# BVE-Reborn/rend3

Hardware: NVIDIA H100
Metric: culled objects/s (fused frustum cull + object-uniform bake) (higher is better)
Workload: dtype f32

## Files before the change

### __graft_entry__.py

```python
import os
import subprocess
import sys

ROOT = os.path.dirname(os.path.abspath(__file__))
CSRC = os.path.join(ROOT, "rend3_b200", "csrc")
OUT = os.path.join(ROOT, "rend3_b200", "librend3_b200.so")
NVCC = os.environ.get("NVCC", "/usr/local/cuda/bin/nvcc")
HOST_CXX = "/usr/bin/g++" if os.path.exists("/usr/bin/g++") else "g++"

SOURCES = [
    ("r3_ctx.cu", ["-fmad=false"]),
    ("r3_cull_bake.cu", ["-fmad=false"]),
    ("r3_tri_cull.cu", ["-fmad=false"]),
    ("r3_raster.cu", ["-fmad=false"]),
    ("r3_shade.cu", []),
    ("r3_batching.cpp", ["-fmad=false"]),
    ("r3_gpu_batching.cu", ["-fmad=false"]),
    ("r3_skinning.cu", ["-fmad=false"]),
    ("r3_animation.cu", ["-fmad=false"]),
    ("r3_object_transforms.cu", ["-fmad=false"]),
    ("r3_mesh_deform.cu", ["-fmad=false"]),
    ("r3_lights.cu", ["-fmad=false"]),
    ("r3_peer.cu", ["-fmad=false"]),
    ("r3_texture_write.cu", ["-fmad=false"]),
]
GENCODE = ["-gencode", "arch=compute_90a,code=sm_90a"]
COMMON = [
    "-std=c++17", "-O3", "-lineinfo", *GENCODE,
    "-ccbin", HOST_CXX, "-Xcompiler", "-fPIC,-fvisibility=hidden,-Wall,-Wno-unused-function",
    "-prec-div=true", "-prec-sqrt=true",
]


def _stale(target, deps):
    if not os.path.exists(target):
        return True
    t = os.path.getmtime(target)
    return any(os.path.getmtime(d) > t for d in deps if os.path.exists(d))


def build(verbose: bool = False) -> None:
    headers = [os.path.join(CSRC, "r3_common.cuh"), os.path.join(CSRC, "r3_scan.cuh"), os.path.join(CSRC, "r3_radix.cuh"), os.path.join(CSRC, "r3_texture.cuh"),
               os.path.join(ROOT, "include", "rend3_b200.h"), os.path.join(ROOT, "include", "r3_layouts.h"), os.path.join(ROOT, "include", "r3_anim_check.h")]
    objs = []
    if os.path.exists(NVCC):
        for src, extra in SOURCES:
            s = os.path.join(CSRC, src)
            o = os.path.join(CSRC, os.path.splitext(src)[0] + ".o")
            objs.append(o)
            if _stale(o, [s] + headers):
                cmd = [NVCC, "-x", "cu", "-c", s, "-o", o] + COMMON + extra + (["-Xptxas", "-v"] if verbose else [])
                r = subprocess.run(cmd, capture_output=True, text=True)
                if verbose or r.returncode != 0:
                    sys.stderr.write(r.stdout + r.stderr)
                if r.returncode != 0:
                    raise RuntimeError(f"nvcc failed on {src}")
        if _stale(OUT, objs):
            cmd = [NVCC, "-shared", "-o", OUT] + objs + GENCODE + ["-ccbin", HOST_CXX, "-lcudart"]
            r = subprocess.run(cmd, capture_output=True, text=True)
            if r.returncode != 0:
                sys.stderr.write(r.stdout + r.stderr)
                raise RuntimeError("link failed")
    elif not os.path.exists(OUT):
        raise RuntimeError("nvcc not found and no prebuilt librend3_b200.so")
    host_src, host_bin = os.path.join(ROOT, "rend3_b200", "host", "r3_frame.cpp"), os.path.join(ROOT, "rend3_b200", "host", "r3_frame")
    if _stale(host_bin, [host_src, OUT, os.path.join(ROOT, "include", "rend3_b200.hpp")] + headers):
        cmd = [HOST_CXX, "-std=c++17", "-O2", "-Wall", "-I", os.path.join(ROOT, "include"), host_src, "-o", host_bin,
               "-L", os.path.join(ROOT, "rend3_b200"), "-lrend3_b200", "-Wl,-rpath,$ORIGIN/.."]
        r = subprocess.run(cmd, capture_output=True, text=True)
        if r.returncode != 0:
            sys.stderr.write(r.stdout + r.stderr)
            raise RuntimeError("host driver build failed")
    sys.path.insert(0, ROOT)
    import oracle
    import oracle.anim
    import oracle.objanim
    import oracle.lights
    import oracle.objtransforms
    import oracle.points

    oracle.build()
    oracle.anim.build()
    oracle.objanim.build()
    oracle.lights.build()
    oracle.objtransforms.build()
    oracle.points.build()
    import rend3_b200


def smoke() -> None:
    sys.path.insert(0, ROOT)
    import numpy as np

    import oracle
    from rend3_b200 import load_cuda_backend
    from rend3_b200.scenes import cube_field_scene
    from rend3_b200.routines import BaseRenderGraph, BaseRenderGraphSettings

    results = {}
    for name, backend in (("cuda", load_cuda_backend(0, parity_target=True)), ("oracle", oracle.load_oracle_backend())):
        ev = cube_field_scene(n_objects=300, seed=7, resolution=(256, 144))
        graph = BaseRenderGraph(backend)
        graph.add_to_graph(ev, (256, 144), 1, BaseRenderGraphSettings(clear_color=(0.1, 0.05, 0.1, 1.0)))
        results[name] = (backend.readback_visible(0xFFFFFFFF).copy(), backend.readback_hdr_f32().copy(), backend.readback_depth().copy())
    vis_c, hdr_c, dep_c = results["cuda"]
    vis_o, hdr_o, dep_o = results["oracle"]
    assert np.array_equal(vis_c, vis_o), "visible-object list differs from the oracle"
    assert np.array_equal(dep_c, dep_o), "depth buffer differs from the oracle"
    err = np.abs(hdr_c - hdr_o) / np.maximum(1.0, np.abs(hdr_o))
    assert err.max() <= 1e-4, f"shaded pixels differ from the oracle by {err.max()}"
    print(f"smoke ok: {len(vis_c)} visible objects, max pixel error {err.max():.2e}")


if __name__ == "__main__":
    build(verbose="-v" in sys.argv)
    print("built", OUT)
```

### rend3_b200/csrc/r3_cull_bake.cu

```cuda
#include <cstdlib>
#include <type_traits>

#include "r3_common.cuh"
#include "r3_scan.cuh"

namespace {

constexpr int CB_THREADS = 256;
constexpr int CB_WARPS = CB_THREADS / 32;
constexpr int CB_WT = 4;
constexpr int CB_CTA_OBJECTS = CB_WARPS * CB_WT * 32;
constexpr int CP_THREADS = 1024;
constexpr int CP_OBJECTS = CP_THREADS * 32;
constexpr int CP_CTAS_PER_TILE = CP_OBJECTS / CB_CTA_OBJECTS;

struct CullBakeParams {
    float view[16];
    float view_proj[16];
    float frustum[5][4];
    uint32_t object_count;
};
struct DeviceCameraParams {
    const r3_camera_header* cam;
    uint32_t object_count;
};
constexpr int CAM_FLOATS = 52;

__global__ void __launch_bounds__(256) split_objects_kernel(const float4* __restrict__ objects, uint32_t n, float* __restrict__ rows_xyz, float* __restrict__ rows_w,
                                                            float4* __restrict__ spheres, float* __restrict__ radii, uint32_t* __restrict__ enabled_bits,
                                                            uint32_t* __restrict__ affine_bits, uint32_t* __restrict__ centre_bits) {
    const int lane = threadIdx.x & 31, k = lane & 7, g = lane >> 3;
    const uint32_t wtile = (blockIdx.x * blockDim.x + threadIdx.x) >> 5, base = wtile * 32u;
    if (base >= n) return;
    uint32_t bits = 0, abits = 0, cbits = 0;
#pragma unroll
    for (int it = 0; it < 8; ++it) {
        const uint32_t obj = base + it * 4 + g;
        float4 r = make_float4(0.f, 0.f, 0.f, 0.f);
        if (obj < n) {
            r = __ldcs(&objects[(size_t)obj * 8 + k]);
            if (k < 4) {
                float* xyz = rows_xyz + (size_t)obj * 12 + k;
                xyz[0] = r.x; xyz[4] = r.y; xyz[8] = r.z;
                rows_w[(size_t)obj * 4 + k] = r.w;
            } else if (k == 4) { spheres[obj] = r; radii[obj] = r.w; }
        }
        const uint32_t b = __ballot_sync(0xFFFFFFFFu, k == 7 && obj < n && __float_as_uint(r.y) != 0u);
        bits |= (((b >> 7) & 1u) | (((b >> 15) & 1u) << 1) | (((b >> 23) & 1u) << 2) | (((b >> 31) & 1u) << 3)) << (it * 4);
        const uint32_t a = __ballot_sync(0xFFFFFFFFu, k < 4 && obj < n && __float_as_uint(r.w) == affine_w_bits(k));
#pragma unroll
        for (int q = 0; q < 4; ++q) abits |= (((a >> (8 * q)) & 0xFu) == 0xFu ? 1u : 0u) << (it * 4 + q);
        const float tx = __shfl_up_sync(0xFFFFFFFFu, r.x, 1), ty = __shfl_up_sync(0xFFFFFFFFu, r.y, 1), tz = __shfl_up_sync(0xFFFFFFFFu, r.z, 1);
        const uint32_t cb = __ballot_sync(0xFFFFFFFFu, k == 4 && obj < n && centre_is_translation(r.x, r.y, r.z, tx, ty, tz));
        cbits |= (((cb >> 4) & 1u) | (((cb >> 12) & 1u) << 1) | (((cb >> 20) & 1u) << 2) | (((cb >> 28) & 1u) << 3)) << (it * 4);
    }
    if (lane == 0) { enabled_bits[wtile] = bits; affine_bits[wtile] = abits; centre_bits[wtile] = cbits; }
}
__global__ void __launch_bounds__(256) split_slots_kernel(const float4* __restrict__ objects, const uint32_t* __restrict__ slots, uint32_t n_updates, uint32_t n_slots,
                                                          float* __restrict__ rows_xyz, float* __restrict__ rows_w, float4* __restrict__ spheres, float* __restrict__ radii,
                                                          uint32_t* __restrict__ enabled_bits, uint32_t* __restrict__ affine_bits, uint32_t* __restrict__ centre_bits) {
    const uint32_t i = (blockIdx.x * blockDim.x + threadIdx.x) >> 3, k = threadIdx.x & 7;
    const uint32_t s = i < n_updates ? slots[i] : n_slots;
    const bool ok = s < n_slots;
    float4 r = make_float4(0.f, 0.f, 0.f, 0.f);
    if (ok) {
        r = objects[(size_t)s * 8 + k];
        if (k < 4) {
            float* xyz = rows_xyz + (size_t)s * 12 + k;
            xyz[0] = r.x; xyz[4] = r.y; xyz[8] = r.z;
            rows_w[(size_t)s * 4 + k] = r.w;
        } else if (k == 4) { spheres[s] = r; radii[s] = r.w; }
    }
    const uint32_t a = __ballot_sync(0xFFFFFFFFu, ok && k < 4 && __float_as_uint(r.w) == affine_w_bits(k));
    const float tx = __shfl_up_sync(0xFFFFFFFFu, r.x, 1), ty = __shfl_up_sync(0xFFFFFFFFu, r.y, 1), tz = __shfl_up_sync(0xFFFFFFFFu, r.z, 1);
    const uint32_t cb = __ballot_sync(0xFFFFFFFFu, ok && k == 4 && centre_is_translation(r.x, r.y, r.z, tx, ty, tz));
    if (ok && k == 7) {
        slot_bit_assign(enabled_bits, s, __float_as_uint(r.y) != 0u);
        slot_bit_assign(affine_bits, s, ((a >> (threadIdx.x & 24u)) & 0xFu) == 0xFu);
        slot_bit_assign(centre_bits, s, (cb >> ((threadIdx.x & 24u) + 4u)) & 1u);
    }
}

template <bool BAKE, bool CULL, bool LIVE, typename Params = CullBakeParams>
__global__ void __launch_bounds__(CB_THREADS)
cull_bake_kernel(const float4* __restrict__ rows_xyz, const float* __restrict__ rows_w, const uint32_t* __restrict__ affine_bits, const float4* __restrict__ spheres,
                 const float* __restrict__ radii, const uint32_t* __restrict__ centre_bits, const uint32_t* __restrict__ enabled_bits, const uint32_t* __restrict__ live_bits, float4* __restrict__ matrices, uint32_t* __restrict__ words,
                 uint32_t* __restrict__ cta_counts, const __grid_constant__ Params p) {
    __shared__ uint32_t s_count[CB_WARPS];
    __shared__ float4 s_rows[BAKE ? CB_WARPS : 1][96];
    const int lane = threadIdx.x & 31, warp = threadIdx.x >> 5;
    const float* view;
    const float* view_proj;
    const float* frustum;
    if constexpr (std::is_same<Params, DeviceCameraParams>::value) {
        __shared__ float s_cam[CAM_FLOATS];
        const float* src = reinterpret_cast<const float*>(p.cam);
        if (threadIdx.x < CAM_FLOATS) s_cam[threadIdx.x] = __ldg(src + (threadIdx.x < 32 ? threadIdx.x : threadIdx.x + 4));
        __syncthreads();
        view = s_cam; view_proj = s_cam + 16; frustum = s_cam + 32;
    } else {
        view = p.view; view_proj = p.view_proj; frustum = &p.frustum[0][0];
    }
    const int col = lane & 3, sub = lane >> 2;
    uint32_t count = 0;
#pragma unroll 2
    for (int wt = 0; wt < CB_WT; ++wt) {
        const uint32_t wtile = (blockIdx.x * CB_WARPS + warp) * CB_WT + wt;
        const uint32_t base = wtile * 32u;
        if (base >= p.object_count) break;
        float4 t[3];
        float4 sp = make_float4(0.f, 0.f, 0.f, 0.f);
        uint32_t enabled = 0u, affine = 0u, centred = 0u;
        if (BAKE && CULL) centred = __ldg(&centre_bits[wtile]);
        if (BAKE) {
#pragma unroll
            for (int q = 0; q < 3; ++q) {
                const uint32_t e = q * 32 + lane;
                t[q] = base + e / 3u < p.object_count ? __ldcs(&rows_xyz[(size_t)base * 3 + e]) : make_float4(0.f, 0.f, 0.f, 0.f);
            }
        }
        const bool centre_from_tile = BAKE && CULL && ((centred >> lane) & 1u);
        if (CULL && base + lane < p.object_count) {
            if (centre_from_tile) sp.w = __ldcs(&radii[base + lane]);
            else sp = __ldcs(&spheres[base + lane]);
        }
        if (BAKE || (CULL && !LIVE)) enabled = __ldg(&enabled_bits[wtile]);
        if (BAKE) affine = __ldg(&affine_bits[wtile]);
        if (BAKE) {
            float4* tile = s_rows[warp];
            __syncwarp();
#pragma unroll
            for (int q = 0; q < 3; ++q) tile[q * 32 + lane] = t[q];
            __syncwarp();
            const float* tf = reinterpret_cast<const float*>(tile);
#pragma unroll
            for (int it = 0; it < 4; ++it) {
                const uint32_t slot = it * 8 + sub, obj = base + slot;
                if (obj < p.object_count && ((enabled >> slot) & 1u)) {
                    const float* c = tf + slot * 12 + col;
                    const float w = ((affine >> slot) & 1u) ? (col == 3 ? 1.0f : 0.0f) : __ldcs(&rows_w[(size_t)obj * 4 + col]);
                    float4* dst = &matrices[(size_t)obj * 8 + col];
                    __stcs(dst, mat_vec_rn(view, c[0], c[4], c[8], w));
                    __stcs(dst + 4, mat_vec_rn(view_proj, c[0], c[4], c[8], w));
                }
            }
        }
        if (CULL) {
            const uint32_t live = LIVE ? __ldg(&live_bits[wtile]) : enabled;
            if constexpr (BAKE) {
                if (centre_from_tile) {
                    const float* tr = reinterpret_cast<const float*>(s_rows[warp]) + lane * 12 + 3;
                    sp.x = tr[0]; sp.y = tr[4]; sp.z = tr[8];
                }
            }
            const float neg_radius = -sp.w;
            bool inside = true;
#pragma unroll
            for (int pl = 0; pl < 5; ++pl) {
                const float* f = frustum + 4 * pl;
                const float d = add_rn(add_rn(add_rn(mul_rn(f[0], sp.x), mul_rn(f[1], sp.y)), mul_rn(f[2], sp.z)), f[3]);
                inside = inside && (d >= neg_radius);
            }
            const uint32_t word = __ballot_sync(0xFFFFFFFFu, base + lane < p.object_count && ((live >> lane) & 1u) && inside);
            if (lane == 0) words[wtile] = word;
            count += __popc(word);
        }
    }
    if (CULL) {
        if (lane == 0) s_count[warp] = count;
        __syncthreads();
        if (threadIdx.x == 0) {
            uint32_t t = 0;
#pragma unroll
            for (int w = 0; w < CB_WARPS; ++w) t += s_count[w];
            cta_counts[blockIdx.x] = t;
        }
    }
}

constexpr uint32_t EX_HEADER_WORDS = 256;
constexpr uint32_t EX_SLOTS = R3_EXCHANGE_SLOTS;
struct ExchangeParams { uint32_t* peers[R3_MAX_EXCHANGE_RANKS]; uint32_t n_ranks, word_offset, words_per_rank, flag_offset, epoch; uint32_t* done; };

__device__ __forceinline__ void st_release_sys(uint32_t* p, uint32_t v) { asm volatile("st.release.sys.global.u32 [%0], %1;" ::"l"(p), "r"(v) : "memory"); }
__device__ __forceinline__ uint32_t ld_acquire_sys(const uint32_t* p) { uint32_t v; asm volatile("ld.acquire.sys.global.u32 %0, [%1];" : "=r"(v) : "l"(p) : "memory"); return v; }

__global__ void __launch_bounds__(CP_THREADS)
compact_visible_kernel(const uint32_t* __restrict__ words, const uint32_t* __restrict__ cta_counts, uint32_t n_words, uint32_t n_cta_counts,
                       uint32_t* __restrict__ visible, uint32_t* __restrict__ visible_count, const __grid_constant__ ExchangeParams ex) {
    __shared__ uint32_t s_warp[CP_THREADS / 32 + 1];
    const uint32_t tile_base = block_sum_u32<CP_THREADS>(cta_counts, min(blockIdx.x * CP_CTAS_PER_TILE, n_cta_counts), s_warp);
    const uint32_t wi = blockIdx.x * CP_THREADS + threadIdx.x;
    const uint32_t word = wi < n_words ? __ldg(&words[wi]) : 0u;
    if (ex.n_ranks && wi < ex.words_per_rank) {
#pragma unroll 1
        for (uint32_t r = 0; r < ex.n_ranks; ++r) ex.peers[r][(size_t)ex.word_offset + wi] = word;
    }
    uint32_t total;
    const uint32_t excl = tile_base + block_scan_excl<CP_THREADS>((uint32_t)__popc(word), s_warp, &total);
    if (threadIdx.x == 0 && blockIdx.x == gridDim.x - 1) *visible_count = tile_base + total;
    warp_expand_words(word, excl, (blockIdx.x * CP_THREADS + (threadIdx.x & ~31u)) * 32u, [&](uint32_t pos, uint32_t id) { visible[pos] = id; });
    if (ex.n_ranks) {
        __syncthreads();
        if (threadIdx.x == 0) {
            __threadfence_system();
            const uint32_t arrived = atomicAdd(ex.done, 1u);
            if (arrived == gridDim.x - 1u) {
                *ex.done = 0u;
                __threadfence_system();
                for (uint32_t r = 0; r < ex.n_ranks; ++r) st_release_sys(ex.peers[r] + ex.flag_offset, ex.epoch);
            }
        }
    }
}

struct MergeParams {
    const uint32_t* gathered;
    uint32_t n_ranks, words_per_rank, parity, epoch, tiles_per_rank;
    uint32_t rank_base[R3_MAX_EXCHANGE_RANKS];
    uint32_t rank_objects[R3_MAX_EXCHANGE_RANKS];
    uint32_t* tile_counts; uint32_t* out; uint32_t* out_count; uint32_t out_cap;
};
__device__ __forceinline__ uint32_t merge_word(const MergeParams& p, uint32_t r, uint32_t w) {
    if (w >= p.words_per_rank) return 0u;
    uint32_t word = __ldcg(p.gathered + EX_HEADER_WORDS + ((size_t)p.parity * p.n_ranks + r) * p.words_per_rank + w);
    const uint32_t n = p.rank_objects[r];
    if (w * 32u >= n) return 0u;
    if (n - w * 32u < 32u) word &= (1u << (n - w * 32u)) - 1u;
    return word;
}
__global__ void exchange_wait_kernel(const uint32_t* __restrict__ flags, uint32_t n_ranks, uint32_t epoch) {
    if (threadIdx.x < n_ranks)
        while ((int32_t)(ld_acquire_sys(flags + threadIdx.x) - epoch) < 0) __nanosleep(100);
}
__global__ void __launch_bounds__(CP_THREADS) exchange_count_kernel(const __grid_constant__ MergeParams p) {
    const uint32_t r = blockIdx.x / p.tiles_per_rank, t = blockIdx.x % p.tiles_per_rank;
    __shared__ uint32_t s_warp[CP_THREADS / 32];
    const uint32_t cnt = block_reduce<CP_THREADS>((uint32_t)__popc(merge_word(p, r, t * CP_THREADS + threadIdx.x)), s_warp);
    if (threadIdx.x == 0) p.tile_counts[blockIdx.x] = cnt;
}
constexpr uint32_t EX_ACK_WORDS = 128;
__global__ void exchange_ack_kernel(const __grid_constant__ ExchangeParams ex, uint32_t epoch) {
    if (threadIdx.x < ex.n_ranks) {
        __threadfence_system();
        st_release_sys(ex.peers[threadIdx.x] + EX_ACK_WORDS + ex.flag_offset, epoch);
    }
}
constexpr uint32_t RC_SLICES = 16;
constexpr int LC_THREADS = 256;
__global__ void __launch_bounds__(LC_THREADS) exchange_light_count_kernel(const __grid_constant__ MergeParams p, uint32_t* __restrict__ out) {
    __shared__ uint32_t s_warp[LC_THREADS / 32];
    const uint32_t r = blockIdx.x / RC_SLICES, sl = blockIdx.x % RC_SLICES;
    const uint32_t n_words = (p.rank_objects[r] + 31u) / 32u;
    const uint32_t vecs = (p.words_per_rank + 3u) / 4u, per = (vecs + RC_SLICES - 1u) / RC_SLICES;
    const uint32_t v0 = sl * per, v1 = min(v0 + per, vecs);
    const uint4* row = reinterpret_cast<const uint4*>(p.gathered + EX_HEADER_WORDS + ((size_t)p.parity * p.n_ranks + r) * p.words_per_rank);
    const uint32_t tail_bits = p.rank_objects[r] & 31u;
    uint32_t cnt = 0;
    for (uint32_t v = v0 + threadIdx.x; v < v1; v += blockDim.x) {
        const uint4 q = __ldcg(&row[v]);
        const uint32_t w[4] = {q.x, q.y, q.z, q.w};
#pragma unroll
        for (uint32_t k = 0; k < 4; ++k) {
            const uint32_t wi = v * 4u + k;
            uint32_t word = wi < n_words ? w[k] : 0u;
            if (tail_bits && wi == n_words - 1u) word &= (1u << tail_bits) - 1u;
            cnt += __popc(word);
        }
    }
    const uint32_t t = block_reduce<LC_THREADS>(cnt, s_warp);
    if (threadIdx.x == 0 && t) { atomicAdd(&out[r], t); atomicAdd(&out[p.n_ranks], t); }
}
__global__ void __launch_bounds__(1024) exchange_rank_counts_kernel(const uint32_t* __restrict__ tile_counts, uint32_t tiles_per_rank, uint32_t n_ranks, uint32_t* __restrict__ out) {
    __shared__ uint32_t s_warp[32];
    uint32_t total = 0;
    for (uint32_t r = 0; r < n_ranks; ++r) {
        const uint32_t sum = block_sum_u32<1024>(tile_counts + r * tiles_per_rank, tiles_per_rank, s_warp);
        if (threadIdx.x == 0) out[r] = sum;
        total += sum;
    }
    if (threadIdx.x == 0) out[n_ranks] = total;
}
__global__ void __launch_bounds__(CP_THREADS) exchange_expand_kernel(const __grid_constant__ MergeParams p) {
    __shared__ uint32_t s_warp[CP_THREADS / 32 + 1];
    const uint32_t r = blockIdx.x / p.tiles_per_rank, t = blockIdx.x % p.tiles_per_rank;
    const uint32_t tile_base = block_sum_u32<CP_THREADS>(p.tile_counts, blockIdx.x, s_warp);
    const uint32_t word = merge_word(p, r, t * CP_THREADS + threadIdx.x);
    uint32_t total;
    const uint32_t excl = tile_base + block_scan_excl<CP_THREADS>((uint32_t)__popc(word), s_warp, &total);
    if (threadIdx.x == 0 && blockIdx.x == gridDim.x - 1) *p.out_count = tile_base + total;
    warp_expand_words(word, excl, p.rank_base[r] + (t * CP_THREADS + (threadIdx.x & ~31u)) * 32u, [&](uint32_t pos, uint32_t id) {
        if (pos < p.out_cap) p.out[pos] = id;
    });
}

}

static int launch_cull_bake(r3_ctx* c, r3_camera* cam, uint32_t mode, const r3_camera_header* d_header) {
    const uint32_t n = cam->header.object_count;
    const bool bake = mode & R3_CB_BAKE, cull = mode & R3_CB_CULL;
    if (n == 0 || (!bake && !cull)) {
        if (cull) R3_CUDA(c, cudaMemsetAsync(cam->d_visible_count, 0, 4, c->stream));
        return R3_OK;
    }
    CullBakeParams p;
    memcpy(p.view, cam->header.view, 64);
    memcpy(p.view_proj, cam->header.view_proj, 64);
    memcpy(p.frustum, cam->header.frustum, 80);
    p.object_count = n;
    const uint32_t n_ctas = (n + CB_CTA_OBJECTS - 1) / CB_CTA_OBJECTS, n_words = (n + 31) / 32;
    const uint64_t set_words = (((uint64_t)n_words + n_ctas + 63) / 64) * 64;
    R3_TRY(r3_reserve_t(c, &cam->d_tile_state, &cam->tile_state_cap, set_words + 2));
    if (cull) cam->words_set ^= 1u;
    uint32_t* words = reinterpret_cast<uint32_t*>(cam->d_tile_state) + (size_t)cam->words_set * set_words;
    cam->d_words = words;
    uint32_t* cta_counts = words + n_words;
    if (!c->hot_valid) return r3_fail(c, R3_E_STATE, "object_uniform_upload before set_objects");
    float4* mats = reinterpret_cast<float4*>(cam->d_matrices);
    const bool live = c->have_live && cull && c->sort_flags.size() >= (size_t)n;
#define R3_CB_LAUNCH(B, C, L) \
    cull_bake_kernel<B, C, L><<<n_ctas, CB_THREADS, 0, c->stream>>>(c->d_hot_xyz, reinterpret_cast<const float*>(c->d_hot_w), c->d_affine_bits, c->d_hot_sphere, \
                                                                    c->d_hot_radius, c->d_centre_bits, c->d_enabled_bits, c->d_live_bits, mats, words, cta_counts, p)
    r3_stage_begin(c, R3_STAGE_CULL_BAKE);
    if (d_header) {
        const DeviceCameraParams dp{d_header, n};
        const uint32_t* live_bits = live ? c->d_live_bits : c->d_enabled_bits;
#define R3_CB_DEV_LAUNCH(B, C)                                                                                                                       \
    cull_bake_kernel<B, C, C, DeviceCameraParams><<<n_ctas, CB_THREADS, 0, c->stream>>>(c->d_hot_xyz, reinterpret_cast<const float*>(c->d_hot_w),     \
                                                                                      c->d_affine_bits, c->d_hot_sphere, c->d_hot_radius, c->d_centre_bits, \
                                                                                      c->d_enabled_bits, live_bits, \
                                                                                      mats, words, cta_counts, dp)
        if (bake && cull) R3_CB_DEV_LAUNCH(true, true);
        else if (bake) R3_CB_DEV_LAUNCH(true, false);
        else R3_CB_DEV_LAUNCH(false, true);
#undef R3_CB_DEV_LAUNCH
    } else if (bake && cull) { if (live) R3_CB_LAUNCH(true, true, true); else R3_CB_LAUNCH(true, true, false); }
    else if (bake) R3_CB_LAUNCH(true, false, false);
    else { if (live) R3_CB_LAUNCH(false, true, true); else R3_CB_LAUNCH(false, true, false); }
#undef R3_CB_LAUNCH
    r3_stage_end(c);
    R3_CHECK_LAUNCH(c, "cull_bake_kernel");
    if (cull) {
        const uint32_t n_tiles = (n_words + CP_THREADS - 1) / CP_THREADS;
        ExchangeParams ex{};
        if (cam->ex_connected) {
            if (n_words > cam->ex_words_per_rank) return r3_fail(c, R3_E_INVALID, "object_uniform_upload: more objects than the exchange was created for");
            for (uint32_t r = 0; r < cam->ex_ranks; ++r) ex.peers[r] = cam->ex_peers[r];
            const uint32_t epoch = ++cam->ex_epoch, parity = epoch % EX_SLOTS;
            if (cam->ex_merge_pending[parity]) {
                R3_CUDA(c, cudaStreamWaitEvent(c->stream, cam->ex_merge_done[parity], 0));
                cam->ex_merge_pending[parity] = false;
            }
            if (epoch > EX_SLOTS && cam->ex_consumed[parity] == epoch - EX_SLOTS) {
                exchange_wait_kernel<<<1, 32, 0, c->stream>>>(cam->d_gathered + EX_ACK_WORDS, cam->ex_ranks, epoch - EX_SLOTS);
                R3_CHECK_LAUNCH(c, "exchange_wait_kernel");
            }
            ex.n_ranks = cam->ex_ranks; ex.words_per_rank = cam->ex_words_per_rank;
            ex.word_offset = EX_HEADER_WORDS + (parity * cam->ex_ranks + cam->ex_rank) * cam->ex_words_per_rank;
            ex.flag_offset = parity * R3_MAX_EXCHANGE_RANKS + cam->ex_rank; ex.epoch = epoch; ex.done = cam->d_ex_done;
            cam->ex_objects = n;
        }
        const uint32_t n_tiles_ex = cam->ex_connected ? (cam->ex_words_per_rank + CP_THREADS - 1) / CP_THREADS : 0u;
        compact_visible_kernel<<<n_tiles > n_tiles_ex ? n_tiles : n_tiles_ex, CP_THREADS, 0, c->stream>>>(words, cta_counts, n_words, n_ctas, cam->d_visible, cam->d_visible_count, ex);
        R3_CHECK_LAUNCH(c, "compact_visible_kernel");
    }
    return R3_OK;
}

int r3_launch_cull_bake(r3_ctx* c, r3_camera* cam, uint32_t mode) { return launch_cull_bake(c, cam, mode, nullptr); }
int r3_launch_cull_bake_device_camera(r3_ctx* c, r3_camera* cam, uint32_t mode, const r3_camera_header* d_header) {
    return launch_cull_bake(c, cam, mode, d_header);
}

uint64_t r3_hot_capacity(uint64_t want) {
    uint64_t cap = 1024;
    while (cap < want) cap *= 2;
    if (cap > want + want / 8 && want > (1u << 20)) cap = want + want / 8;
    return cap;
}
int r3_split_objects(r3_ctx* c) {
    const uint32_t n = c->n_slots;
    const uint64_t want = n ? n : 1;
    if (want > c->hot_cap) {
        cudaFree(c->d_hot_xyz); cudaFree(c->d_hot_w); cudaFree(c->d_hot_sphere); cudaFree(c->d_enabled_bits); cudaFree(c->d_affine_bits);
        cudaFree(c->d_hot_radius); cudaFree(c->d_centre_bits);
        c->d_hot_xyz = nullptr; c->d_hot_w = nullptr; c->d_hot_sphere = nullptr; c->d_enabled_bits = nullptr; c->d_affine_bits = nullptr;
        c->d_hot_radius = nullptr; c->d_centre_bits = nullptr; c->hot_cap = 0;
        const uint64_t cap = r3_hot_capacity(want);
        R3_CUDA(c, cudaMalloc((void**)&c->d_hot_xyz, cap * 48));
        R3_CUDA(c, cudaMalloc((void**)&c->d_hot_w, cap * 16));
        R3_CUDA(c, cudaMalloc((void**)&c->d_hot_sphere, cap * 16));
        R3_CUDA(c, cudaMalloc((void**)&c->d_hot_radius, cap * 4));
        R3_CUDA(c, cudaMalloc((void**)&c->d_enabled_bits, ((cap + 31) / 32 + 1) * 4));
        R3_CUDA(c, cudaMalloc((void**)&c->d_affine_bits, ((cap + 31) / 32 + 1) * 4));
        R3_CUDA(c, cudaMalloc((void**)&c->d_centre_bits, ((cap + 31) / 32 + 1) * 4));
        c->hot_cap = cap;
    }
    if (n) {
        const uint32_t warps = (n + 31) / 32;
        split_objects_kernel<<<(warps + 7) / 8, 256, 0, c->stream>>>(reinterpret_cast<const float4*>(c->d_objects), n, reinterpret_cast<float*>(c->d_hot_xyz),
                                                                      reinterpret_cast<float*>(c->d_hot_w), c->d_hot_sphere, c->d_hot_radius, c->d_enabled_bits,
                                                                      c->d_affine_bits, c->d_centre_bits);
        R3_CHECK_LAUNCH(c, "split_objects_kernel");
    }
    c->hot_valid = true;
    return R3_OK;
}
int r3_split_slots(r3_ctx* c, const uint32_t* d_slots, uint32_t n) {
    if (!c->hot_valid || n == 0) return R3_OK;
    split_slots_kernel<<<(n * 8 + 255) / 256, 256, 0, c->stream>>>(reinterpret_cast<const float4*>(c->d_objects), d_slots, n, c->n_slots,
                                                                    reinterpret_cast<float*>(c->d_hot_xyz), reinterpret_cast<float*>(c->d_hot_w), c->d_hot_sphere,
                                                                    c->d_hot_radius, c->d_enabled_bits, c->d_affine_bits, c->d_centre_bits);
    R3_CHECK_LAUNCH(c, "split_slots_kernel");
    return R3_OK;
}
namespace {
__global__ void mask_word_kernel(uint32_t* word_a, uint32_t* word_b, uint32_t* word_c, uint32_t keep_mask) {
    if (word_a) *word_a &= keep_mask;
    if (word_b) *word_b &= keep_mask;
    if (word_c) *word_c &= keep_mask;
}
}
int r3_launch_mask_word(r3_ctx* c, uint32_t* word_a, uint32_t* word_b, uint32_t* word_c, uint32_t keep_mask) {
    mask_word_kernel<<<1, 1, 0, c->stream>>>(word_a, word_b, word_c, keep_mask);
    R3_CHECK_LAUNCH(c, "mask_word_kernel");
    return R3_OK;
}
int r3_grow_hot(r3_ctx* c, uint32_t old_n, uint32_t n) {
    if (!c->hot_valid) old_n = 0;
    const uint64_t old_words = ((uint64_t)old_n + 31) / 32;
    if ((uint64_t)n > c->hot_cap || !c->d_hot_xyz) {
        const uint64_t cap = r3_hot_capacity(n ? n : 1), bit_words = (cap + 31) / 32 + 1;
        float4 *xyz = nullptr, *w = nullptr, *sph = nullptr;
        float* rad = nullptr;
        uint32_t *en = nullptr, *af = nullptr, *ce = nullptr;
        R3_CUDA(c, cudaMalloc((void**)&xyz, cap * 48));
        R3_CUDA(c, cudaMalloc((void**)&w, cap * 16));
        R3_CUDA(c, cudaMalloc((void**)&sph, cap * 16));
        R3_CUDA(c, cudaMalloc((void**)&rad, cap * 4));
        R3_CUDA(c, cudaMalloc((void**)&en, bit_words * 4));
        R3_CUDA(c, cudaMalloc((void**)&af, bit_words * 4));
        R3_CUDA(c, cudaMalloc((void**)&ce, bit_words * 4));
        if (old_n) {
            R3_CUDA(c, cudaMemcpyAsync(xyz, c->d_hot_xyz, (size_t)old_n * 48, cudaMemcpyDeviceToDevice, c->stream));
            R3_CUDA(c, cudaMemcpyAsync(w, c->d_hot_w, (size_t)old_n * 16, cudaMemcpyDeviceToDevice, c->stream));
            R3_CUDA(c, cudaMemcpyAsync(sph, c->d_hot_sphere, (size_t)old_n * 16, cudaMemcpyDeviceToDevice, c->stream));
            R3_CUDA(c, cudaMemcpyAsync(rad, c->d_hot_radius, (size_t)old_n * 4, cudaMemcpyDeviceToDevice, c->stream));
            R3_CUDA(c, cudaMemcpyAsync(en, c->d_enabled_bits, old_words * 4, cudaMemcpyDeviceToDevice, c->stream));
            R3_CUDA(c, cudaMemcpyAsync(af, c->d_affine_bits, old_words * 4, cudaMemcpyDeviceToDevice, c->stream));
            R3_CUDA(c, cudaMemcpyAsync(ce, c->d_centre_bits, old_words * 4, cudaMemcpyDeviceToDevice, c->stream));
        }
        R3_CUDA(c, r3_stream_sync(c));
        cudaFree(c->d_hot_xyz); cudaFree(c->d_hot_w); cudaFree(c->d_hot_sphere); cudaFree(c->d_enabled_bits); cudaFree(c->d_affine_bits);
        cudaFree(c->d_hot_radius); cudaFree(c->d_centre_bits);
        c->d_hot_xyz = xyz; c->d_hot_w = w; c->d_hot_sphere = sph; c->d_enabled_bits = en; c->d_affine_bits = af; c->hot_cap = cap;
        c->d_hot_radius = rad; c->d_centre_bits = ce;
    }
    const uint64_t first_word = old_n / 32, new_words = ((uint64_t)n + 31) / 32;
    if (n > old_n) {
        R3_CUDA(c, cudaMemsetAsync(c->d_hot_xyz + (size_t)old_n * 3, 0, (size_t)(n - old_n) * 48, c->stream));
        R3_CUDA(c, cudaMemsetAsync(c->d_hot_w + old_n, 0, (size_t)(n - old_n) * 16, c->stream));
        R3_CUDA(c, cudaMemsetAsync(c->d_hot_sphere + old_n, 0, (size_t)(n - old_n) * 16, c->stream));
        R3_CUDA(c, cudaMemsetAsync(c->d_hot_radius + old_n, 0, (size_t)(n - old_n) * 4, c->stream));
    }
    const uint64_t whole = (old_n & 31u) ? first_word + 1 : first_word;
    if (new_words > whole) {
        R3_CUDA(c, cudaMemsetAsync(c->d_enabled_bits + whole, 0, (new_words - whole) * 4, c->stream));
        R3_CUDA(c, cudaMemsetAsync(c->d_affine_bits + whole, 0, (new_words - whole) * 4, c->stream));
        R3_CUDA(c, cudaMemsetAsync(c->d_centre_bits + whole, 0, (new_words - whole) * 4, c->stream));
    }
    if (old_n & 31u)
        R3_TRY(r3_launch_mask_word(c, c->d_enabled_bits + first_word, c->d_affine_bits + first_word, c->d_centre_bits + first_word, (1u << (old_n & 31u)) - 1u));
    c->hot_valid = true;
    return R3_OK;
}

R3_EXPORT int r3_exchange_create(r3_ctx* c, uint32_t camera, uint32_t n_ranks, uint32_t my_rank, uint32_t max_objects_per_rank, uint8_t handle_out[R3_IPC_HANDLE_BYTES]) {
    if (!c || !handle_out) return r3_fail(c, R3_E_INVALID, "exchange_create: null");
    if (n_ranks == 0 || n_ranks > R3_MAX_EXCHANGE_RANKS || my_rank >= n_ranks || max_objects_per_rank == 0) return r3_fail(c, R3_E_INVALID, "exchange_create: bad rank layout");
    r3_camera* cam = r3_get_camera(c, camera);
    if (!cam) return r3_fail(c, R3_E_INVALID, "exchange_create: bad camera");
    static_assert(sizeof(cudaIpcMemHandle_t) == R3_IPC_HANDLE_BYTES, "IPC handle size");
    cudaSetDevice(c->device);
    if (cam->d_gathered) return r3_fail(c, R3_E_STATE, "exchange_create: already created for this camera");
    const uint32_t wpr = (((max_objects_per_rank + 31u) / 32u) + 63u) & ~63u;
    const size_t total_words = EX_HEADER_WORDS + (size_t)EX_SLOTS * n_ranks * wpr;
    R3_CUDA(c, cudaMalloc((void**)&cam->d_gathered, total_words * 4));
    R3_CUDA(c, cudaMemsetAsync(cam->d_gathered, 0, total_words * 4, c->stream));
    if (!cam->d_ex_done) R3_CUDA(c, cudaMalloc((void**)&cam->d_ex_done, 16));
    R3_CUDA(c, cudaMemsetAsync(cam->d_ex_done, 0, 16, c->stream));
    R3_CUDA(c, r3_stream_sync(c));
    cam->ex_epoch = 0; cam->ex_objects = 0;
    for (auto& e : cam->ex_consumed) e = 0;
    cudaIpcMemHandle_t h;
    R3_CUDA(c, cudaIpcGetMemHandle(&h, cam->d_gathered));
    memcpy(handle_out, &h, sizeof h);
    cam->ex_ranks = n_ranks; cam->ex_rank = my_rank; cam->ex_words_per_rank = wpr; cam->ex_connected = false;
    return R3_OK;
}
R3_EXPORT int r3_exchange_connect(r3_ctx* c, uint32_t camera, const uint8_t* handles) {
    if (!c || !handles) return r3_fail(c, R3_E_INVALID, "exchange_connect: null");
    r3_camera* cam = r3_get_camera(c, camera);
    if (!cam || !cam->d_gathered) return r3_fail(c, R3_E_STATE, "exchange_connect before exchange_create");
    cudaSetDevice(c->device);
    for (uint32_t r = 0; r < cam->ex_ranks; ++r) {
        if (r == cam->ex_rank) { cam->ex_peers[r] = cam->d_gathered; continue; }
        cudaIpcMemHandle_t h;
        memcpy(&h, handles + (size_t)r * R3_IPC_HANDLE_BYTES, sizeof h);
        void* p = nullptr;
        R3_CUDA(c, cudaIpcOpenMemHandle(&p, h, cudaIpcMemLazyEnablePeerAccess));
        cam->ex_peers[r] = (uint32_t*)p;
    }
    cam->ex_connected = true;
    return R3_OK;
}
R3_EXPORT int r3_exchange_words(r3_ctx* c, uint32_t camera, void** device_ptr, uint64_t* nbytes, uint32_t* words_per_rank) {
    if (!c || !device_ptr || !nbytes) return r3_fail(c, R3_E_INVALID, "exchange_words: null");
    r3_camera* cam = r3_get_camera(c, camera);
    if (!cam || !cam->d_gathered) return r3_fail(c, R3_E_STATE, "exchange_words before exchange_create");
    *device_ptr = cam->d_gathered + EX_HEADER_WORDS + (size_t)(cam->ex_epoch % EX_SLOTS) * cam->ex_ranks * cam->ex_words_per_rank;
    *nbytes = (uint64_t)cam->ex_ranks * cam->ex_words_per_rank * 4;
    if (words_per_rank) *words_per_rank = cam->ex_words_per_rank;
    return R3_OK;
}
static int r3_exchange_consume(r3_ctx* c, uint32_t camera, const uint32_t* rank_objects, const uint32_t* rank_base, bool expand);
R3_EXPORT int r3_exchange_merge(r3_ctx* c, uint32_t camera, const uint32_t* rank_objects, const uint32_t* rank_base) {
    return r3_exchange_consume(c, camera, rank_objects, rank_base, true);
}
static int r3_exchange_consume(r3_ctx* c, uint32_t camera, const uint32_t* rank_objects, const uint32_t* rank_base, bool expand) {
    if (!c || !rank_objects) return r3_fail(c, R3_E_INVALID, "exchange_merge: null");
    r3_camera* cam = r3_get_camera(c, camera);
    if (!cam || !cam->d_gathered || !cam->ex_connected) return r3_fail(c, R3_E_STATE, "exchange_merge before exchange_connect");
    if (cam->ex_epoch == 0) return r3_fail(c, R3_E_STATE, "exchange_merge before the first cull of the exchange");
    cudaSetDevice(c->device);
    MergeParams p{};
    uint64_t total = 0;
    for (uint32_t r = 0; r < cam->ex_ranks; ++r) {
        if ((rank_objects[r] + 31u) / 32u > cam->ex_words_per_rank) return r3_fail(c, R3_E_INVALID, "exchange_merge: a shard is larger than the exchange was created for");
        p.rank_objects[r] = rank_objects[r];
        p.rank_base[r] = rank_base ? rank_base[r] : r * cam->ex_words_per_rank * 32u;
        total += rank_objects[r];
    }
    if (total >= (1ull << 32)) return r3_fail(c, R3_E_INVALID, "exchange_merge: more than 2^32 objects");
    p.gathered = cam->d_gathered; p.n_ranks = cam->ex_ranks; p.words_per_rank = cam->ex_words_per_rank;
    p.epoch = cam->ex_epoch; p.parity = cam->ex_epoch % EX_SLOTS;
    p.tiles_per_rank = (cam->ex_words_per_rank + CP_THREADS - 1) / CP_THREADS;
    const uint32_t n_tiles = p.tiles_per_rank * cam->ex_ranks;
    if (expand) R3_TRY(r3_reserve_t(c, &cam->d_global_visible, &cam->global_visible_cap, total + 1));
    R3_TRY(r3_reserve_t(c, &cam->d_merge_counts, &cam->merge_counts_cap, (uint64_t)n_tiles + 32));
    p.tile_counts = cam->d_merge_counts + 32; p.out = cam->d_global_visible; p.out_count = cam->d_merge_counts; p.out_cap = (uint32_t)total;
    if (!c->side_stream) {
        int lo = 0, hi = 0;
        cudaDeviceGetStreamPriorityRange(&lo, &hi);
        R3_CUDA(c, cudaStreamCreateWithPriority(&c->side_stream, cudaStreamNonBlocking, lo));
    }
    const int slot = (int)(cam->ex_epoch % EX_SLOTS);
    if (!cam->ex_cull_done[slot]) R3_CUDA(c, cudaEventCreateWithFlags(&cam->ex_cull_done[slot], cudaEventDisableTiming));
    if (!cam->ex_merge_done[slot]) R3_CUDA(c, cudaEventCreateWithFlags(&cam->ex_merge_done[slot], cudaEventDisableTiming));
    R3_CUDA(c, cudaEventRecord(cam->ex_cull_done[slot], c->stream));
    R3_CUDA(c, cudaStreamWaitEvent(c->side_stream, cam->ex_cull_done[slot], 0));
    exchange_wait_kernel<<<1, 32, 0, c->side_stream>>>(cam->d_gathered + p.parity * R3_MAX_EXCHANGE_RANKS, cam->ex_ranks, p.epoch);
    R3_CHECK_LAUNCH(c, "exchange_wait_kernel");
    if (!expand) {
        R3_CUDA(c, cudaMemsetAsync(cam->d_merge_counts + 8, 0, ((size_t)cam->ex_ranks + 1) * 4, c->side_stream));
        exchange_light_count_kernel<<<cam->ex_ranks * RC_SLICES, LC_THREADS, 0, c->side_stream>>>(p, cam->d_merge_counts + 8);
        R3_CHECK_LAUNCH(c, "exchange_light_count_kernel");
    } else {
        exchange_count_kernel<<<n_tiles, CP_THREADS, 0, c->side_stream>>>(p);
        R3_CHECK_LAUNCH(c, "exchange_count_kernel");
        exchange_rank_counts_kernel<<<1, 1024, 0, c->side_stream>>>(p.tile_counts, p.tiles_per_rank, cam->ex_ranks, cam->d_merge_counts + 8);
        R3_CHECK_LAUNCH(c, "exchange_rank_counts_kernel");
        exchange_expand_kernel<<<n_tiles, CP_THREADS, 0, c->side_stream>>>(p);
        R3_CHECK_LAUNCH(c, "exchange_expand_kernel");
    }
    {
        ExchangeParams ack{};
        for (uint32_t r = 0; r < cam->ex_ranks; ++r) ack.peers[r] = cam->ex_peers[r];
        ack.n_ranks = cam->ex_ranks; ack.flag_offset = cam->ex_rank;
        exchange_ack_kernel<<<1, 32, 0, c->side_stream>>>(ack, cam->ex_epoch);
        R3_CHECK_LAUNCH(c, "exchange_ack_kernel");
    }
    R3_CUDA(c, cudaEventRecord(cam->ex_merge_done[slot], c->side_stream));
    cam->ex_merge_pending[slot] = true;
    cam->ex_consumed[slot] = cam->ex_epoch;
    return R3_OK;
}
R3_EXPORT int r3_exchange_count(r3_ctx* c, uint32_t camera, const uint32_t* rank_objects) {
    return r3_exchange_consume(c, camera, rank_objects, nullptr, false);
}
R3_EXPORT int r3_exchange_counts(r3_ctx* c, uint32_t camera, uint32_t* counts ) {
    if (!c || !counts) return r3_fail(c, R3_E_INVALID, "exchange_counts: null");
    r3_camera* cam = r3_get_camera(c, camera);
    if (!cam || !cam->d_merge_counts) return r3_fail(c, R3_E_STATE, "exchange_counts before exchange_count / exchange_merge");
    cudaSetDevice(c->device);
    for (int k = 0; k < (int)EX_SLOTS; ++k)
        if (cam->ex_merge_pending[k]) { R3_CUDA(c, cudaStreamWaitEvent(c->stream, cam->ex_merge_done[k], 0)); cam->ex_merge_pending[k] = false; }
    R3_CUDA(c, cudaMemcpyAsync(counts, cam->d_merge_counts + 8, ((size_t)cam->ex_ranks + 1) * 4, cudaMemcpyDeviceToHost, c->stream));
    R3_CUDA(c, r3_stream_sync(c));
    return R3_OK;
}
R3_EXPORT int r3_exchange_merged(r3_ctx* c, uint32_t camera, void** device_list, void** device_count, uint64_t* capacity) {
    if (!c || !device_list || !device_count) return r3_fail(c, R3_E_INVALID, "exchange_merged: null");
    r3_camera* cam = r3_get_camera(c, camera);
    if (!cam || !cam->d_global_visible) return r3_fail(c, R3_E_STATE, "exchange_merged before exchange_merge");
    for (int k = 0; k < (int)EX_SLOTS; ++k)
        if (cam->ex_merge_pending[k]) { R3_CUDA(c, cudaStreamWaitEvent(c->stream, cam->ex_merge_done[k], 0)); cam->ex_merge_pending[k] = false; }
    *device_list = cam->d_global_visible; *device_count = cam->d_merge_counts;
    if (capacity) *capacity = cam->global_visible_cap;
    return R3_OK;
}
R3_EXPORT int r3_exchange_destroy(r3_ctx* c, uint32_t camera) {
    if (!c) return R3_E_INVALID;
    r3_camera* cam = r3_get_camera(c, camera);
    if (!cam) return r3_fail(c, R3_E_INVALID, "exchange_destroy: bad camera");
    cudaSetDevice(c->device);
    r3_stream_sync(c);
    for (uint32_t r = 0; r < cam->ex_ranks; ++r)
        if (cam->ex_connected && r != cam->ex_rank && cam->ex_peers[r]) cudaIpcCloseMemHandle(cam->ex_peers[r]);
    if (c->side_stream) cudaStreamSynchronize(c->side_stream);
    for (int k = 0; k < (int)EX_SLOTS; ++k) {
        if (cam->ex_cull_done[k]) cudaEventDestroy(cam->ex_cull_done[k]);
        if (cam->ex_merge_done[k]) cudaEventDestroy(cam->ex_merge_done[k]);
        cam->ex_cull_done[k] = cam->ex_merge_done[k] = nullptr; cam->ex_merge_pending[k] = false;
    }
    cudaFree(cam->d_gathered);
    cam->d_gathered = nullptr; cam->ex_connected = false; cam->ex_ranks = 0; cam->ex_epoch = 0;
    for (auto& p : cam->ex_peers) p = nullptr;
    return R3_OK;
}
```

Measured before the change: 14.85 billion.

## Stage baked matrices in shared memory and write them out with bulk async copies

The bake path now writes each warp's view and view-projection matrices into a per-warp shared-memory tile. Lane 0 then issues TMA bulk copies (cp.async.bulk) of contiguous enabled runs to global memory, replacing per-thread streaming stores. Launch bounds now request 4 CTAs per SM for the bake variants. A standalone HBM bandwidth probe kernel is also added for measuring store paths. The aim is fully coalesced, asynchronous 128-byte-row writes, at the cost of extra shared memory, which may cap occupancy, and a wait on the previous bulk group before the staging tile is reused.

```diff
diff --git a/__graft_entry__.py b/__graft_entry__.py
--- a/__graft_entry__.py
+++ b/__graft_entry__.py
@@ -23,6 +23,7 @@
     ("r3_lights.cu", ["-fmad=false"]),
     ("r3_peer.cu", ["-fmad=false"]),
     ("r3_texture_write.cu", ["-fmad=false"]),
+    ("r3_hbm_probe.cu", []),
 ]
 GENCODE = ["-gencode", "arch=compute_90a,code=sm_90a"]
 COMMON = [
diff --git a/rend3_b200/csrc/r3_cull_bake.cu b/rend3_b200/csrc/r3_cull_bake.cu
--- a/rend3_b200/csrc/r3_cull_bake.cu
+++ b/rend3_b200/csrc/r3_cull_bake.cu
@@ -82,12 +82,13 @@
 }
 
 template <bool BAKE, bool CULL, bool LIVE, typename Params = CullBakeParams>
-__global__ void __launch_bounds__(CB_THREADS)
+__global__ void __launch_bounds__(CB_THREADS, BAKE ? 4 : 0)
 cull_bake_kernel(const float4* __restrict__ rows_xyz, const float* __restrict__ rows_w, const uint32_t* __restrict__ affine_bits, const float4* __restrict__ spheres,
                  const float* __restrict__ radii, const uint32_t* __restrict__ centre_bits, const uint32_t* __restrict__ enabled_bits, const uint32_t* __restrict__ live_bits, float4* __restrict__ matrices, uint32_t* __restrict__ words,
                  uint32_t* __restrict__ cta_counts, const __grid_constant__ Params p) {
     __shared__ uint32_t s_count[CB_WARPS];
     __shared__ float4 s_rows[BAKE ? CB_WARPS : 1][96];
+    __shared__ float4 s_mats[BAKE ? CB_WARPS : 1][BAKE ? 32 * 8 : 1];
     const int lane = threadIdx.x & 31, warp = threadIdx.x >> 5;
     const float* view;
     const float* view_proj;
@@ -133,16 +134,32 @@
             for (int q = 0; q < 3; ++q) tile[q * 32 + lane] = t[q];
             __syncwarp();
             const float* tf = reinterpret_cast<const float*>(tile);
+            float4* out = s_mats[warp];
+            if (lane == 0) asm volatile("cp.async.bulk.wait_group.read 0;" ::: "memory");
+            __syncwarp();
 #pragma unroll
             for (int it = 0; it < 4; ++it) {
                 const uint32_t slot = it * 8 + sub, obj = base + slot;
                 if (obj < p.object_count && ((enabled >> slot) & 1u)) {
                     const float* c = tf + slot * 12 + col;
                     const float w = ((affine >> slot) & 1u) ? (col == 3 ? 1.0f : 0.0f) : __ldcs(&rows_w[(size_t)obj * 4 + col]);
-                    float4* dst = &matrices[(size_t)obj * 8 + col];
-                    __stcs(dst, mat_vec_rn(view, c[0], c[4], c[8], w));
-                    __stcs(dst + 4, mat_vec_rn(view_proj, c[0], c[4], c[8], w));
+                    out[slot * 8 + col] = mat_vec_rn(view, c[0], c[4], c[8], w);
+                    out[slot * 8 + 4 + col] = mat_vec_rn(view_proj, c[0], c[4], c[8], w);
                 }
+            }
+            asm volatile("fence.proxy.async.shared::cta;" ::: "memory");
+            __syncwarp();
+            if (lane == 0) {
+                const uint32_t left = p.object_count - base;
+                uint32_t m = enabled & (left < 32u ? (1u << left) - 1u : 0xFFFFFFFFu);
+                while (m) {
+                    const uint32_t first = __ffs(m) - 1u, len = __ffs(~(m >> first)) ? __ffs(~(m >> first)) - 1u : 32u - first;
+                    asm volatile("cp.async.bulk.global.shared::cta.bulk_group [%0], [%1], %2;"
+                                 ::"l"(matrices + (size_t)(base + first) * 8), "r"((uint32_t)__cvta_generic_to_shared(out + first * 8)), "r"(len * 128u)
+                                 : "memory");
+                    m &= ~(len == 32u ? 0xFFFFFFFFu : ((1u << len) - 1u) << first);
+                }
+                asm volatile("cp.async.bulk.commit_group;" ::: "memory");
             }
         }
         if (CULL) {
@@ -166,6 +183,7 @@
             count += __popc(word);
         }
     }
+    if (BAKE && lane == 0) asm volatile("cp.async.bulk.wait_group.read 0;" ::: "memory");
     if (CULL) {
         if (lane == 0) s_count[warp] = count;
         __syncthreads();
diff --git a/rend3_b200/csrc/r3_hbm_probe.cu b/rend3_b200/csrc/r3_hbm_probe.cu
--- /dev/null
+++ b/rend3_b200/csrc/r3_hbm_probe.cu
@@ -0,0 +1,98 @@
+#include <algorithm>
+
+#include "r3_common.cuh"
+
+namespace {
+
+constexpr int HP_THREADS = 256, HP_WARPS = HP_THREADS / 32, HP_WT = 4;
+constexpr uint32_t HP_TILE_BYTES = 32 * 128;
+enum : uint32_t { R3_PROBE_MEMCPY = 0, R3_PROBE_MIX = 1, R3_PROBE_BULK = 2, R3_PROBE_BULK_WAVES = 3 };
+
+__device__ __forceinline__ float4 probe_value(const float4 t[3], float r, int k) {
+    float4 v = t[k % 3];
+    if (k == 7) v.w = r;
+    return v;
+}
+
+template <bool BULK>
+__global__ void __launch_bounds__(HP_THREADS) hbm_probe_kernel(const float4* __restrict__ rows, const float* __restrict__ radii, float4* __restrict__ out, uint32_t n, bool waves) {
+    extern __shared__ __align__(128) float4 s_out[];
+    const int lane = threadIdx.x & 31, warp = threadIdx.x >> 5;
+    const uint32_t first = waves ? blockIdx.x * HP_WARPS + warp : (blockIdx.x * HP_WARPS + warp) * HP_WT, step = waves ? gridDim.x * HP_WARPS : 1u;
+    const uint32_t n_tiles = n / 32u;
+    for (uint32_t wt = 0, wtile = first; wtile < n_tiles && (waves || wt < HP_WT); ++wt, wtile += step) {
+        const uint32_t base = wtile * 32u;
+        float4 t[3];
+#pragma unroll
+        for (int q = 0; q < 3; ++q) t[q] = __ldcs(&rows[(size_t)base * 3 + q * 32 + lane]);
+        const float r = __ldcs(&radii[base + lane]);
+        float4* dst = out + (size_t)base * 8;
+        if constexpr (!BULK) {
+#pragma unroll
+            for (int k = 0; k < 8; ++k) __stcs(&dst[k * 32 + lane], probe_value(t, r, k));
+        } else {
+            float4* buf = s_out + (warp * 2 + (wt & 1)) * 256;
+            if (lane == 0 && wt >= 2) asm volatile("cp.async.bulk.wait_group.read 1;" ::: "memory");
+            __syncwarp();
+#pragma unroll
+            for (int k = 0; k < 8; ++k) buf[k * 32 + lane] = probe_value(t, r, k);
+            asm volatile("fence.proxy.async.shared::cta;" ::: "memory");
+            __syncwarp();
+            if (lane == 0) {
+                asm volatile("cp.async.bulk.global.shared::cta.bulk_group [%0], [%1], %2;" ::"l"(dst), "r"((uint32_t)__cvta_generic_to_shared(buf)), "r"(HP_TILE_BYTES)
+                             : "memory");
+                asm volatile("cp.async.bulk.commit_group;" ::: "memory");
+            }
+        }
+    }
+    if constexpr (BULK) {
+        if (lane == 0) asm volatile("cp.async.bulk.wait_group.read 0;" ::: "memory");
+    }
+}
+
+}
+
+R3_EXPORT int r3_hbm_probe(uint32_t probe, const void* d_in, void* d_out, uint64_t n, uint32_t launches, float* ms_out) {
+    if (!d_in || !d_out || !ms_out || launches == 0 || n < 32 || n > (1ull << 31) || probe > R3_PROBE_BULK_WAVES) return R3_E_INVALID;
+    n &= ~31ull;
+    cudaStream_t s = nullptr;
+    cudaEvent_t e0 = nullptr, e1 = nullptr;
+    int rc = R3_E_CUDA;
+    uint32_t ctas = (uint32_t)((n + HP_WARPS * HP_WT * 32 - 1) / (HP_WARPS * HP_WT * 32));
+    const bool bulk = probe == R3_PROBE_BULK || probe == R3_PROBE_BULK_WAVES, waves = probe == R3_PROBE_BULK_WAVES;
+    const size_t smem = bulk ? (size_t)HP_WARPS * 2 * HP_TILE_BYTES : 0;
+    int dev = 0, sms = 0, per_sm = 0;
+    const float4* rows = static_cast<const float4*>(d_in);
+    const float* radii = reinterpret_cast<const float*>(static_cast<const char*>(d_in) + n * 48);
+    float4* out = static_cast<float4*>(d_out);
+    auto launch = [&]() {
+        if (probe == R3_PROBE_MEMCPY) return cudaMemcpyAsync(d_out, d_in, n * 90, cudaMemcpyDeviceToDevice, s);
+        if (!bulk) hbm_probe_kernel<false><<<ctas, HP_THREADS, 0, s>>>(rows, radii, out, (uint32_t)n, false);
+        else hbm_probe_kernel<true><<<ctas, HP_THREADS, smem, s>>>(rows, radii, out, (uint32_t)n, waves);
+        return cudaGetLastError();
+    };
+    if (cudaStreamCreateWithFlags(&s, cudaStreamNonBlocking) != cudaSuccess || cudaEventCreate(&e0) != cudaSuccess || cudaEventCreate(&e1) != cudaSuccess) goto done;
+    if (smem && cudaFuncSetAttribute(hbm_probe_kernel<true>, cudaFuncAttributeMaxDynamicSharedMemorySize, (int)smem) != cudaSuccess) goto done;
+    if (waves) {
+        if (cudaGetDevice(&dev) != cudaSuccess || cudaDeviceGetAttribute(&sms, cudaDevAttrMultiProcessorCount, dev) != cudaSuccess ||
+            cudaOccupancyMaxActiveBlocksPerMultiprocessor(&per_sm, hbm_probe_kernel<true>, HP_THREADS, smem) != cudaSuccess || per_sm < 1)
+            goto done;
+        ctas = std::min<uint32_t>(ctas, (uint32_t)(sms * per_sm));
+    }
+    for (int i = 0; i < 3; ++i)
+        if (launch() != cudaSuccess) goto done;
+    if (cudaEventRecord(e0, s) != cudaSuccess) goto done;
+    for (uint32_t i = 0; i < launches; ++i)
+        if (launch() != cudaSuccess) goto done;
+    if (cudaEventRecord(e1, s) != cudaSuccess || cudaEventSynchronize(e1) != cudaSuccess) goto done;
+    if (cudaEventElapsedTime(ms_out, e0, e1) != cudaSuccess) goto done;
+    *ms_out /= (float)launches;
+    rc = R3_OK;
+done:
+    if (s) cudaStreamSynchronize(s);
+    if (e0) cudaEventDestroy(e0);
+    if (e1) cudaEventDestroy(e1);
+    if (s) cudaStreamDestroy(s);
+    if (rc != R3_OK) cudaGetLastError();
+    return rc;
+}
```

Measured after the change: 15.23 billion (median of 6 runs). +2.5%, better.
